# HeyWeCome/WhisprRec

Hardware: AMD Instinct MI355X
Metric: BPR training triplets/sec (higher is better)
Workload: dtype f32; 1 GPU; BPRMF emb_size=64, synthetic 1000000 users x 1000000 items (uniform ids), batch 65536, SGD l2=0, plan build in timed region; batch=65536, emb_size=64, optimizer=SGD, plan_chunk_batches=64, tables=single GPU, step_stream=whisprrec_amd.hip_ops.PipelinedSgd, plan=group plan (no per-batch sort: flags + lists of the shared rows, wr_group.hip), chained_step_launch=True, plan_build=on a side stream, beside the steps of the chunk before

## Files before the change

whisprrec_amd/csrc/wr_group.hip:

```cpp
#include "wr_common.h"
#include <hip/hip_ext.h>

#include <algorithm>

namespace wr {

constexpr int kGpThreads = 1024;
constexpr unsigned kGpRangeBits = 18;
constexpr int kGpWords = 1 << (kGpRangeBits - 5);
constexpr int kGpCap = 8192;
constexpr int kGpBins = 4096;
constexpr int kGpMaxBin = 256;
constexpr int kGpMaxRanges = 8;
constexpr int64_t kGpMaxBatch = 1 << 17;
constexpr int kGpLongRun = 64;
constexpr int kGpMetaWords = 16;
#ifndef WR_GP_DBG
#define WR_GP_DBG 0
#endif

struct GroupLayout {
    int64_t nb, B, fw;
    int R_u, R_i, cap_u, cap_i;
    unsigned mask_u, mask_i, hbits_u, hbits_i;
    int64_t flags, ucnt, icnt, ul_row, ul_src, il_row, il_src, total;
    int64_t zero_words;
};

static inline int ranges_for(int64_t n_rows, unsigned *mask, unsigned *hbits, int *cap) {
    unsigned bits = kGpRangeBits;
    while (bits < kGpRangeBits + 3 && (int64_t(1) << bits) < n_rows) ++bits;
    *mask = (1u << bits) - 1u;
    *hbits = bits;
    const int R = 1 << (bits - kGpRangeBits);
    *cap = kGpCap;
    return R;
}

static bool group_layout(int64_t n, int64_t B, int64_t n_users, int64_t n_items, GroupLayout &L) {
    if (n <= 0 || n >= (int64_t(1) << 31) || B <= 0 || B > kGpMaxBatch) return false;
    if (n_users <= 0 || n_users >= (int64_t(1) << 31) || n_items <= 0 || n_items >= (int64_t(1) << 31)) return false;
    L.nb = (n + B - 1) / B;
    L.B = B;
    L.fw = (B + 31) / 32;
    L.R_u = ranges_for(n_users, &L.mask_u, &L.hbits_u, &L.cap_u);
    L.R_i = ranges_for(n_items, &L.mask_i, &L.hbits_i, &L.cap_i);
    L.flags = kGpMetaWords;
    L.ucnt = L.flags + L.nb * L.fw * 4;
    L.icnt = L.ucnt + align_up(L.nb * L.R_u, 4);
    L.zero_words = L.icnt + align_up(L.nb * L.R_i, 4);
    L.ul_row = L.zero_words;
    L.ul_src = L.ul_row + L.nb * L.R_u * (int64_t)L.cap_u;
    L.il_row = L.ul_src + L.nb * L.R_u * (int64_t)L.cap_u;
    L.il_src = L.il_row + L.nb * L.R_i * (int64_t)L.cap_i;
    L.total = L.il_src + L.nb * L.R_i * (int64_t)L.cap_i;
    return true;
}

struct GpDev {
    int *meta;
    unsigned *flags;
    int *ucnt, *icnt;
    int *ul_row, *ul_src, *il_row, *il_src;
    int R_u, R_i, cap_u, cap_i;
    unsigned mask_u, mask_i, hbits_u, hbits_i;
    int fw;
};

static inline GpDev group_dev(int32_t *plan, const GroupLayout &L) {
    return GpDev{plan, reinterpret_cast<unsigned *>(plan + L.flags), plan + L.ucnt, plan + L.icnt, plan + L.ul_row,
                 plan + L.ul_src, plan + L.il_row, plan + L.il_src, L.R_u, L.R_i, L.cap_u, L.cap_i, L.mask_u, L.mask_i,
                 L.hbits_u, L.hbits_i, (int)L.fw};
}

template <typename F>
__device__ __forceinline__ void gp_scan(const int *__restrict__ a, int cnt, F f) {
    if ((reinterpret_cast<uintptr_t>(a) & 15u) == 0) {
        const int n4 = cnt >> 2;
        const int4 *a4 = reinterpret_cast<const int4 *>(a);
        int i = threadIdx.x;
        for (; i + 3 * kGpThreads < n4; i += 4 * kGpThreads) {
            int4 v[4];
#pragma unroll
            for (int q = 0; q < 4; ++q) v[q] = a4[i + q * kGpThreads];
#pragma unroll
            for (int q = 0; q < 4; ++q) {
                const int at = 4 * (i + q * kGpThreads);
                f(v[q].x, at);
                f(v[q].y, at + 1);
                f(v[q].z, at + 2);
                f(v[q].w, at + 3);
            }
        }
        for (; i < n4; i += kGpThreads) {
            const int4 v = a4[i];
            f(v.x, 4 * i);
            f(v.y, 4 * i + 1);
            f(v.z, 4 * i + 2);
            f(v.w, 4 * i + 3);
        }
        for (int j = (n4 << 2) + threadIdx.x; j < cnt; j += kGpThreads) f(a[j], j);
    } else {
        for (int j = threadIdx.x; j < cnt; j += kGpThreads) f(a[j], j);
    }
}

__global__ __launch_bounds__(kGpThreads) void group_plan_kernel(const int *__restrict__ u, const int *__restrict__ p,
                                                                 const int *__restrict__ n, int64_t n_total, int B, int nb,
                                                                 int n_users, int n_items, GpDev L) {
    extern __shared__ __attribute__((aligned(16))) unsigned gp_lds[];
    unsigned *seen = gp_lds;
    unsigned long long *keys = reinterpret_cast<unsigned long long *>(gp_lds);
    unsigned *multi = gp_lds + 2 * kGpCap;
    unsigned *f0 = multi + kGpWords, *f1 = f0 + L.fw, *f2 = f1 + L.fw;
    int &n_list = *reinterpret_cast<int *>(f2 + L.fw);
    const int per = L.R_u + L.R_i;
    const unsigned lb = xcd_contiguous_id(blockIdx.x, gridDim.x);
    const int b = (int)(lb / (unsigned)per), rr = (int)(lb % (unsigned)per);
    const bool item = rr >= L.R_u;
    const unsigned r = (unsigned)(item ? rr - L.R_u : rr);
    const int64_t base = (int64_t)b * B;
    const int Bb = (int)((base + B <= n_total) ? B : (n_total - base));
    const unsigned n_rows = (unsigned)(item ? n_items : n_users);
    const unsigned mask = item ? L.mask_i : L.mask_u;
    const unsigned rb = (item ? L.hbits_i : L.hbits_u) - kGpRangeBits, rsel = (1u << rb) - 1u;
    for (int i = threadIdx.x; i < kGpWords; i += kGpThreads) {
        seen[i] = 0u;
        multi[i] = 0u;
    }
    for (int i = threadIdx.x; i < 3 * L.fw; i += kGpThreads) f0[i] = 0u;
    if (threadIdx.x == 0) n_list = 0;
    __syncthreads();
    auto mark = [&](int row, int) {
        if ((unsigned)row >= n_rows) {
            L.meta[0] = 1;
            return;
        }
        const unsigned h = (unsigned)row & mask;
        if ((h & rsel) != r) return;
        const unsigned bit = h >> rb, m = 1u << (bit & 31u);
        const unsigned old = atomicOr(&seen[bit >> 5], m);
        if (old & m) atomicOr(&multi[bit >> 5], m);
    };
    if (!(WR_GP_DBG & 8)) {
        if (item) {
            gp_scan(p + base, Bb, mark);
            gp_scan(n + base, Bb, mark);
        } else {
            gp_scan(u + base, Bb, mark);
        }
    }
    __syncthreads();
    auto several = [&](int row) -> bool {
        const unsigned h = (unsigned)row & mask;
        if ((h & rsel) != r) return false;
        const unsigned bit = h >> rb;
        return (multi[bit >> 5] >> (bit & 31u)) & 1u;
    };
    auto append = [&](int row, unsigned src) {
        const int pos = atomicAdd(&n_list, 1);
        if (pos < kGpCap) keys[pos] = ((unsigned long long)(unsigned)row << 32) | src;
    };
    if (!(WR_GP_DBG & 2)) {
        const bool next = b + 1 < nb && !(WR_GP_DBG & 16);
        const int64_t nbase = base + B;
        const int Bn = next ? (int)((nbase + B <= n_total) ? B : (n_total - nbase)) : 0;
        auto defer = [&](int row, int t) {
            if (several(row)) atomicOr(&f2[t >> 5], 1u << (t & 31));
        };
        if (item) {
            gp_scan(p + base, Bb, [&](int row, int t) {
                if (several(row)) {
                    atomicOr(&f0[t >> 5], 1u << (t & 31));
                    append(row, (unsigned)t << 1);
                }
            });
            gp_scan(n + base, Bb, [&](int row, int t) {
                if (several(row)) {
                    atomicOr(&f1[t >> 5], 1u << (t & 31));
                    append(row, ((unsigned)t << 1) | 1u);
                }
            });
            gp_scan(p + nbase, Bn, defer);
            gp_scan(n + nbase, Bn, defer);
        } else {
            gp_scan(u + base, Bb, [&](int row, int t) {
                if (several(row)) {
                    atomicOr(&f0[t >> 5], 1u << (t & 31));
                    append(row, (unsigned)t << 1);
                }
            });
            gp_scan(u + nbase, Bn, defer);
        }
    }
    __syncthreads();
    if (!(WR_GP_DBG & 4)) {
        unsigned *fb = L.flags + (int64_t)b * L.fw * 4;
        for (int w = threadIdx.x; w < L.fw; w += kGpThreads) {
            if (f0[w]) __hip_atomic_fetch_or(fb + 4 * w + (item ? 1 : 0), f0[w], __ATOMIC_RELAXED, __HIP_MEMORY_SCOPE_AGENT);
            if (item && f1[w]) __hip_atomic_fetch_or(fb + 4 * w + 2, f1[w], __ATOMIC_RELAXED, __HIP_MEMORY_SCOPE_AGENT);
            if (f2[w])
                __hip_atomic_fetch_or(fb + 4 * (L.fw + w) + 3, f2[w], __ATOMIC_RELAXED, __HIP_MEMORY_SCOPE_AGENT);
        }
    }
    const int cap = item ? L.cap_i : L.cap_u, R = item ? L.R_i : L.R_u;
    int m = n_list;
    if (m > cap) {
        if (threadIdx.x == 0) L.meta[1] = 1;
        m = cap;
    }
    int *cnt = reinterpret_cast<int *>(multi);
    unsigned short *out16 = reinterpret_cast<unsigned short *>(multi + kGpBins);
    int *wave_tot = reinterpret_cast<int *>(f0);
    auto bin_of = [&](unsigned long long k) -> int { return (int)(((((unsigned)(k >> 32)) & mask) >> rb) & (kGpBins - 1)); };
    int *lrow = (item ? L.il_row : L.ul_row) + ((int64_t)b * R + r) * cap, *lsrc = (item ? L.il_src : L.ul_src) + ((int64_t)b * R + r) * cap;
    __syncthreads();
    for (int i = threadIdx.x; i < kGpBins; i += kGpThreads) cnt[i] = 0;
    __syncthreads();
    if (!(WR_GP_DBG & 1)) {
        for (int j = threadIdx.x; j < m; j += kGpThreads) atomicAdd(&cnt[bin_of(keys[j])], 1);
        __syncthreads();
        constexpr int kOwn = kGpBins / kGpThreads;
        const int c0 = (int)threadIdx.x * kOwn;
        int local = 0;
#pragma unroll
        for (int j = 0; j < kOwn; ++j) local += cnt[c0 + j];
        int incl = local;
#pragma unroll
        for (int d = 1; d < 64; d <<= 1) {
            const int v = __shfl_up(incl, d, 64);
            if ((int)(threadIdx.x & 63) >= d) incl += v;
        }
        if ((threadIdx.x & 63) == 63) wave_tot[threadIdx.x >> 6] = incl;
        __syncthreads();
        int run = incl - local;
        for (int w = 0; w < (int)(threadIdx.x >> 6); ++w) run += wave_tot[w];
#pragma unroll
        for (int j = 0; j < kOwn; ++j) {
            const int c = cnt[c0 + j];
            cnt[c0 + j] = run;
            run += c;
        }
        __syncthreads();
        for (int j = threadIdx.x; j < m; j += kGpThreads) out16[atomicAdd(&cnt[bin_of(keys[j])], 1)] = (unsigned short)j;
        __syncthreads();
        for (int j = threadIdx.x; j < m; j += kGpThreads) {
            const unsigned long long k = keys[j];
            const int bin = bin_of(k);
            const int lo = bin ? cnt[bin - 1] : 0, hi = cnt[bin];
            if (hi - lo > kGpMaxBin) {
                L.meta[1] = 1;
                continue;
            }
            int pos = lo, same = 0;
            for (int jj = lo; jj < hi; ++jj) {
                const unsigned long long o = keys[out16[jj]];
                pos += o < k ? 1 : 0;
                same += (unsigned)(o >> 32) == (unsigned)(k >> 32) ? 1 : 0;
            }
            if (same > kGpLongRun) L.meta[2] = 1;
            lrow[pos] = (int)(k >> 32);
            lsrc[pos] = (int)(unsigned)k;
        }
    } else {
        for (int j = threadIdx.x; j < m; j += kGpThreads) {
            lrow[j] = (int)(keys[j] >> 32);
            lsrc[j] = (int)(unsigned)keys[j];
        }
    }
    if (threadIdx.x == 0) (item ? L.icnt : L.ucnt)[(int64_t)b * R + r] = m;
}

__global__ __launch_bounds__(kBlock) void narrow_ids_kernel(const int64_t *__restrict__ u, const int64_t *__restrict__ p,
                                                             const int64_t *__restrict__ n, int *__restrict__ u32,
                                                             int *__restrict__ p32, int *__restrict__ n32, int64_t cnt) {
    const int64_t i = (int64_t)blockIdx.x * kBlock + threadIdx.x;
    if (i >= cnt) return;
    const int64_t a = u[i], b = p[i], c = n[i];
    u32[i] = (a >= 0 && a < (int64_t(1) << 31)) ? (int)a : -1;
    p32[i] = (b >= 0 && b < (int64_t(1) << 31)) ? (int)b : -1;
    n32[i] = (c >= 0 && c < (int64_t(1) << 31)) ? (int)c : -1;
}

constexpr int kGsTile = 32;
constexpr int kGsAhead = 8;
constexpr int kGsShards = 64;
constexpr int kGsShardStride = 16;
constexpr int kGsStepWords = kGsShards * kGsShardStride;
constexpr int kGsDefChunk = 32;
constexpr int kGsLdsInts = 1024 + 8;
constexpr unsigned kGsSpinLimit = 1u << 22;

struct GsBatch {
    const int *u, *p, *n;
    const uint4 *flags;
    const int *ul_row, *ul_src, *ul_cnt, *il_row, *il_src, *il_cnt;
    int B, R_u, R_i, cap_u, cap_i;
};

struct GsArgs {
    float *U, *I;
    int D;
    float lr;
    GsBatch cur;
    float *Z, *ZU, *partials;
    float denom;
    GsBatch prev;
    const float *Zp, *ZUp, *partials_prev;
    int n_partials_prev;
    float denom_prev;
    float *loss_prev;
    int nA, nIT, nUT, nDS, tiles_at, side_at;
    int chained;
    unsigned *done, *timeout;
    float *Gs;
    int nL;
};

template <int NV>
__device__ __forceinline__ Row<NV> row_zero() {
    Row<NV> r;
#pragma unroll
    for (int k = 0; k < NV; ++k) r.v[k] = make_float4(0.f, 0.f, 0.f, 0.f);
    return r;
}

template <int T, int NV, bool FULL>
__device__ __forceinline__ void gs_single(const GsArgs &a, int t, int u, int p, int n, bool us, bool ps, bool ns, int lane,
                                          float &terms) {
    const Row<NV> ur = load_row<T, NV, FULL>(a.U, u, a.D, lane);
    const Row<NV> pr = load_row<T, NV, FULL>(a.I, p, a.D, lane);
    const Row<NV> nr = load_row<T, NV, FULL>(a.I, n, a.D, lane);
    const float sp = team_sum<T>(dot_partial<NV>(ur, pr));
    const float sn = team_sum<T>(dot_partial<NV>(ur, nr));
    float term, c;
    bpr_terms(sp, sn, a.denom, term, c);
    terms += term;
    Row<NV> g, z;
#pragma unroll
    for (int k = 0; k < NV; ++k) {
        g.v[k] = make_float4(c * (pr.v[k].x - nr.v[k].x), c * (pr.v[k].y - nr.v[k].y), c * (pr.v[k].z - nr.v[k].z),
                             c * (pr.v[k].w - nr.v[k].w));
        z.v[k] = make_float4(c * ur.v[k].x, c * ur.v[k].y, c * ur.v[k].z, c * ur.v[k].w);
    }
    const float lr = a.lr;
    if (!us) {
        Row<NV> w;
#pragma unroll
        for (int k = 0; k < NV; ++k)
            w.v[k] = make_float4(ur.v[k].x - lr * g.v[k].x, ur.v[k].y - lr * g.v[k].y, ur.v[k].z - lr * g.v[k].z,
                                 ur.v[k].w - lr * g.v[k].w);
        store_row<T, NV, FULL>(a.U, u, a.D, lane, w);
    } else {
        store_row<T, NV, FULL>(a.ZU, t, a.D, lane, g);
    }
    if (!ps) {
        if (a.Gs != nullptr && p >= a.nL) {
            store_row<T, NV, FULL>(a.Gs, p - a.nL, a.D, lane, z);
        } else {
            Row<NV> w;
#pragma unroll
            for (int k = 0; k < NV; ++k)
                w.v[k] = make_float4(pr.v[k].x - lr * z.v[k].x, pr.v[k].y - lr * z.v[k].y, pr.v[k].z - lr * z.v[k].z,
                                     pr.v[k].w - lr * z.v[k].w);
            store_row<T, NV, FULL>(a.I, p, a.D, lane, w);
        }
    }
    if (!ns) {
        if (a.Gs != nullptr && n >= a.nL) {
            Row<NV> zn;
#pragma unroll
            for (int k = 0; k < NV; ++k) zn.v[k] = make_float4(-z.v[k].x, -z.v[k].y, -z.v[k].z, -z.v[k].w);
            store_row<T, NV, FULL>(a.Gs, n - a.nL, a.D, lane, zn);
        } else {
            Row<NV> w;
#pragma unroll
            for (int k = 0; k < NV; ++k)
                w.v[k] = make_float4(nr.v[k].x - lr * (-z.v[k].x), nr.v[k].y - lr * (-z.v[k].y), nr.v[k].z - lr * (-z.v[k].z),
                                     nr.v[k].w - lr * (-z.v[k].w));
            store_row<T, NV, FULL>(a.I, n, a.D, lane, w);
        }
    }
    if (ps || ns) store_row<T, NV, FULL>(a.Z, t, a.D, lane, z);
}

__device__ __forceinline__ void gs_wait_tiles(const GsArgs &a) {
    if (threadIdx.x < 64) {
        const int j = (int)threadIdx.x;
        const int n_sig = a.nIT + a.nUT;
        const unsigned want = j < kGsShards ? (unsigned)((n_sig - j + kGsShards - 1) / kGsShards) : 0u;
        const unsigned *shard = a.done + (j < kGsShards ? j : 0) * kGsShardStride;
        unsigned spins = 0;
        for (;;) {
            const bool ok = __hip_atomic_load(shard, __ATOMIC_RELAXED, __HIP_MEMORY_SCOPE_AGENT) >= want;
            if (__all(ok)) break;
            __builtin_amdgcn_s_sleep(8);
            if (++spins > kGsSpinLimit) {
                if (j == 0) __hip_atomic_store(a.timeout, 1u, __ATOMIC_RELAXED, __HIP_MEMORY_SCOPE_AGENT);
                break;
            }
        }
        __builtin_amdgcn_fence(__ATOMIC_ACQUIRE, "agent");
        asm volatile("s_waitcnt vmcnt(0)" ::: "memory");
    }
    __syncthreads();
}

__device__ __forceinline__ bool gs_tile_of(const int *__restrict__ cnt, int R, int cap, int q, int &seg, int &e0, int &len) {
    int c[kGpMaxRanges];
#pragma unroll
    for (int s = 0; s < kGpMaxRanges; ++s) c[s] = cnt[s < R ? s : 0];
    asm volatile("" : "+v"(c[0]), "+v"(c[1]), "+v"(c[2]), "+v"(c[3]), "+v"(c[4]), "+v"(c[5]), "+v"(c[6]), "+v"(c[7]));
#pragma unroll
    for (int s = 0; s < kGpMaxRanges; ++s)
        if (s >= R) c[s] = 0;
    bool found = false;
#pragma unroll
    for (int s = 0; s < kGpMaxRanges; ++s) {
        const int cs = min(c[s], cap);
        const int nt = (cs + kGsTile - 1) / kGsTile;
        if (!found && q < nt) {
// ... 240 lines not shown
#if WR_GS_DBG & 8
        f = make_uint4(0u, 0u, 0u, 0u);
#endif
        asm volatile("" : "+v"(u), "+v"(p), "+v"(n), "+v"(f.x), "+v"(f.y), "+v"(f.z), "+v"(f.w));
        const unsigned bit = 1u << (t & 31);
        if (t < a.cur.B && !(a.chained && (f.w & bit)))
            gs_single<T, NV, FULL>(a, t, u, p, n, f.x & bit, f.y & bit, f.z & bit, lane, terms);
        slot = b;
    }
    if (lane != 0) terms = 0.f;
    const float sum = block_sum(terms, scratch);
    if (threadIdx.x == 0) a.partials[slot] = sum;
}

static inline int64_t gs_ws_one(int64_t B, int32_t D) {
    const int64_t nA = (B + teams_per_block(D) - 1) / teams_per_block(D);
    return 2 * align_up(B * (int64_t)D * 4, 256) + align_up((nA + 512) * 4, 256);
}

#ifndef WR_GS_TILES_AT
#define WR_GS_TILES_AT 0
#endif
#ifndef WR_GS_SIDE_AT
#define WR_GS_SIDE_AT 12
#endif
#ifndef WR_GS_NUT
#define WR_GS_NUT 256
#endif
#ifndef WR_GS_NDS
#define WR_GS_NDS 64
#endif
#ifndef WR_GS_NIT
#define WR_GS_NIT 1024
#endif

struct GroupRun {
    TablePair tabs;
    const int32_t *u, *p, *n, *plan;
    int64_t n_triplets, batch_size, plan_words, workspace_bytes, sync_words;
    BatchRange range;
    float lr, *loss_out;
    void *const *events;
    void *workspace;
    uint32_t *sync;
    int n_cu;
    float *grad_slots;
    int64_t n_local_items, global_batch;
    hipStream_t stream;
};

template <int T, int NV, bool FULL>
static int32_t launch_group_steps(const GroupRun &g, const GroupLayout &L, const GpDev &G) {
    const int32_t D = g.tabs.D;
    const int64_t n_batches = g.range.n_batches, global_batch = g.global_batch;
    uint32_t *const sync = g.sync;
    const int64_t B = L.B;
    const int64_t ws_one = gs_ws_one(B, D), zb = align_up(B * (int64_t)D * 4, 256);
    char *ws = reinterpret_cast<char *>(g.workspace);
    float *Zs[2] = {reinterpret_cast<float *>(ws), reinterpret_cast<float *>(ws + ws_one)};
    float *ZUs[2] = {reinterpret_cast<float *>(ws + zb), reinterpret_cast<float *>(ws + ws_one + zb)};
    float *Ps[2] = {reinterpret_cast<float *>(ws + 2 * zb), reinterpret_cast<float *>(ws + ws_one + 2 * zb)};
    constexpr int TEAMS = kBlock / T;
    WR_HIP(hipMemsetAsync(sync, 0, (size_t)(n_batches * kGsStepWords) * 4, g.stream));
    uint32_t *timeout = sync + (g.sync_words - 4);
    int nDS = WR_GS_NDS;
    while (nDS > g.n_cu / 4 && nDS > 1) nDS >>= 1;
    auto batch_of = [&](int64_t b) {
        const int64_t off = b * B;
        const int Bk = (int)batch_len(g.n_triplets, B, b);
        return GsBatch{g.u + off, g.p + off, g.n + off, reinterpret_cast<const uint4 *>(G.flags + b * L.fw * 4),
                       G.ul_row + b * L.R_u * (int64_t)L.cap_u, G.ul_src + b * L.R_u * (int64_t)L.cap_u, G.ucnt + b * L.R_u,
                       G.il_row + b * L.R_i * (int64_t)L.cap_i, G.il_src + b * L.R_i * (int64_t)L.cap_i, G.icnt + b * L.R_i,
                       Bk, L.R_u, L.R_i, L.cap_u, L.cap_i};
    };
    auto ev = [&](int64_t k, int j) { return g.events ? reinterpret_cast<hipEvent_t>(g.events[2 * k + j]) : (hipEvent_t) nullptr; };
    int n_partials_prev = 0;
    for (int64_t k = 0; k <= n_batches; ++k) {
        GsArgs a{};
        a.U = g.tabs.U;
        a.I = g.tabs.I;
        a.D = D;
        a.lr = g.lr;
        a.done = sync + (k < n_batches ? k : 0) * kGsStepWords;
        a.timeout = timeout;
        a.Gs = g.grad_slots;
        a.nL = (int)g.n_local_items;
        const bool have_cur = k < n_batches, have_prev = k > 0;
        if (have_cur) {
            a.cur = batch_of(g.range.first_batch + k);
            a.Z = Zs[k & 1];
            a.ZU = ZUs[k & 1];
            a.partials = Ps[k & 1];
            a.denom = global_batch > 0 ? (float)global_batch : (float)a.cur.B;
            a.nA = (int)((a.cur.B + TEAMS - 1) / TEAMS);
            a.nDS = have_prev ? nDS : 0;
            a.chained = have_prev ? 1 : 0;
        }
        if (have_prev) {
            a.prev = batch_of(g.range.first_batch + k - 1);
            a.Zp = Zs[(k - 1) & 1];
            a.ZUp = ZUs[(k - 1) & 1];
            a.partials_prev = Ps[(k - 1) & 1];
            a.n_partials_prev = n_partials_prev;
            a.denom_prev = global_batch > 0 ? (float)global_batch : (float)a.prev.B;
            a.loss_prev = at_or_null(g.loss_out, k - 1);
            a.nIT = (int)std::min<int64_t>(WR_GS_NIT, (2 * B + kGsTile - 1) / kGsTile + L.R_i);
            a.nUT = (int)std::min<int64_t>(WR_GS_NUT, (B + kGsTile - 1) / kGsTile + L.R_u);
        }
        a.tiles_at = (int)((int64_t)a.nA * WR_GS_TILES_AT / 16);
        a.side_at = std::max(a.tiles_at, (int)((int64_t)a.nA * WR_GS_SIDE_AT / 16));
        const dim3 grid((unsigned)(a.nA + a.nIT + a.nUT + a.nDS));
        hipEvent_t e0 = have_cur ? ev(k, 0) : nullptr, e1 = have_cur ? ev(k, 1) : nullptr;
        if (e0 != nullptr || e1 != nullptr)
            hipExtLaunchKernelGGL((bprmf_group_step<T, NV, FULL>), grid, dim3(kBlock), 0, g.stream, e0, e1, 0, a);
        else
            hipLaunchKernelGGL((bprmf_group_step<T, NV, FULL>), grid, dim3(kBlock), 0, g.stream, a);
        WR_LAUNCH_CHECK("bprmf_group_step");
        n_partials_prev = a.nA + a.nDS;
    }
    return WR_OK;
}

static int32_t check_group_plan(const char *entry, const GroupRun &g, GroupLayout &L) {
    int32_t rc;
    if ((rc = check_whole_lines(entry, whole_lines(g.tabs.U, g.tabs.I, g.tabs.D), g.tabs.D)) != WR_OK) return rc;
    WR_REQUIRE(group_layout(g.n_triplets, g.batch_size, g.tabs.n_users, g.tabs.n_items, L), WR_E_RANGE,
               "group plan not applicable to n=%lld, batch=%lld", (long long)g.n_triplets, (long long)g.batch_size);
    WR_REQUIRE(g.plan_words >= L.total, WR_E_WORKSPACE, "group plan: %lld words < %lld", (long long)g.plan_words, (long long)L.total);
    return WR_OK;
}

static int32_t run_group(const char *entry, GroupRun &g, const GroupLayout &L, int64_t sync_batches) {
    int32_t rc;
    if ((rc = check_workspace(entry, g.workspace, g.workspace_bytes, 2 * gs_ws_one(g.batch_size, g.tabs.D))) != WR_OK) return rc;
    if ((rc = check_sync_words(entry, g.sync, g.sync_words, sync_batches * kGsStepWords + 4)) != WR_OK) return rc;
    if (g.range.n_batches == 0) return WR_OK;
    if (g.n_cu == 0 && (rc = device_cu_count(&g.n_cu)) != WR_OK) return rc;
    const GpDev G = group_dev(const_cast<int32_t *>(g.plan), L);
#define WR_CALL_GS(T_, NV_, FULL_) return launch_group_steps<T_, NV_, FULL_>(g, L, G)
    WR_DISPATCH_D(g.tabs.D, WR_CALL_GS);
#undef WR_CALL_GS
    return WR_OK;
}

}

using namespace wr;

extern "C" {

int64_t wr_group_plan_words(int64_t n_triplets, int64_t batch_size, int64_t n_users, int64_t n_items) {
    GroupLayout L;
    if (!group_layout(n_triplets, batch_size, n_users, n_items, L)) return 0;
    return L.total;
}

int32_t wr_group_plan_layout(int64_t n_triplets, int64_t batch_size, int64_t n_users, int64_t n_items, int64_t *out) {
    WR_REQUIRE(out != nullptr, WR_E_NULL, "out is NULL");
    GroupLayout L;
    WR_REQUIRE(group_layout(n_triplets, batch_size, n_users, n_items, L), WR_E_RANGE,
               "group plan not applicable to n=%lld, batch=%lld", (long long)n_triplets, (long long)batch_size);
    const int64_t v[16] = {L.nb, L.fw, L.R_u, L.R_i, (int64_t)L.mask_u, (int64_t)L.mask_i, L.flags, L.ucnt, L.icnt, L.ul_row,
                           L.ul_src, L.il_row, L.il_src, L.total, L.cap_u, L.cap_i};
    for (int i = 0; i < 16; ++i) out[i] = v[i];
    return WR_OK;
}

int32_t wr_narrow_ids_i64(const int64_t *u, const int64_t *p, const int64_t *n, int32_t *u32, int32_t *p32, int32_t *n32,
                          int64_t count, void *stream_) {
    WR_REQUIRE(u && p && n && u32 && p32 && n32, WR_E_NULL, "index arrays must not be NULL");
    WR_REQUIRE(count >= 0 && count < (int64_t(1) << 40), WR_E_SHAPE, "count out of range");
    if (count == 0) return WR_OK;
    hipLaunchKernelGGL(narrow_ids_kernel, dim3((unsigned)((count + kBlock - 1) / kBlock)), dim3(kBlock), 0,
                       reinterpret_cast<hipStream_t>(stream_), u, p, n, u32, p32, n32, count);
    WR_LAUNCH_CHECK("narrow_ids_kernel");
    return WR_OK;
}

int32_t wr_group_plan_build(const int32_t *u, const int32_t *p, const int32_t *n, int64_t n_triplets, int64_t batch_size,
                            int64_t n_users, int64_t n_items, int32_t *plan, int64_t plan_words, void *stream_) {
    WR_REQUIRE(u && p && n && plan, WR_E_NULL, "index arrays / plan must not be NULL");
    GroupLayout L;
    WR_REQUIRE(group_layout(n_triplets, batch_size, n_users, n_items, L), WR_E_RANGE,
               "group plan not applicable to n=%lld, batch=%lld", (long long)n_triplets, (long long)batch_size);
    WR_REQUIRE(aligned16(plan) && plan_words >= L.total, WR_E_WORKSPACE, "group plan: %lld words < %lld", (long long)plan_words,
               (long long)L.total);
    WR_REQUIRE(L.nb * (L.R_u + L.R_i) < (int64_t(1) << 31), WR_E_SHAPE, "group plan: too many batches in one plan");
    hipStream_t stream = reinterpret_cast<hipStream_t>(stream_);
    WR_HIP(hipMemsetAsync(plan, 0, (size_t)L.zero_words * 4, stream));
    const size_t lds = (size_t)(2 * kGpCap + kGpWords + 3 * L.fw + 4) * 4;
    static bool attr_set = false;
    if (!attr_set) {
        WR_HIP(hipFuncSetAttribute(reinterpret_cast<const void *>(group_plan_kernel), hipFuncAttributeMaxDynamicSharedMemorySize,
                                   (int)((2 * kGpCap + kGpWords + 3 * ((kGpMaxBatch + 31) / 32) + 4) * 4)));
        attr_set = true;
    }
    const GpDev G = group_dev(plan, L);
    hipLaunchKernelGGL(group_plan_kernel, dim3((unsigned)(L.nb * (L.R_u + L.R_i))), dim3(kGpThreads), lds, stream, u, p, n,
                       n_triplets, (int)batch_size, (int)L.nb, (int)n_users, (int)n_items, G);
    WR_LAUNCH_CHECK("group_plan_kernel");
    return WR_OK;
}

int64_t wr_bprmf_group_workspace_bytes(int64_t batch_size, int32_t D) { return 2 * gs_ws_one(batch_size, D); }

int64_t wr_bprmf_group_sync_words(int64_t n_batches) { return n_batches < 0 ? WR_E_SHAPE : (n_batches + 1) * kGsStepWords + 4; }

int32_t wr_bprmf_group_supported(const float *user_tab, const float *item_tab, int32_t D) {
    return (user_tab && item_tab && D >= 4 && D <= 1024 && D % 4 == 0 && whole_lines(user_tab, item_tab, D)) ? 1 : 0;
}

int32_t wr_bprmf_run_sgd_group(float *user_tab, int64_t n_users, float *item_tab, int64_t n_items, int32_t D,
                               const int32_t *u, const int32_t *p, const int32_t *n, int64_t n_triplets, int64_t batch_size,
                               const int32_t *plan, int64_t plan_words, int64_t first_batch, int64_t n_batches, float lr,
                               float *loss_out, void *const *events, void *workspace, int64_t workspace_bytes, int32_t *sync,
                               int64_t sync_words, void *stream) {
    GroupRun g{};
    g.tabs = TablePair{user_tab, item_tab, n_users, n_items, D};
    g.u = u; g.p = p; g.n = n; g.n_triplets = n_triplets; g.batch_size = batch_size;
    g.plan = plan; g.plan_words = plan_words;
    g.range = BatchRange{first_batch, n_batches};
    g.lr = lr; g.loss_out = loss_out; g.events = events;
    g.workspace = workspace; g.workspace_bytes = workspace_bytes;
    g.sync = reinterpret_cast<uint32_t *>(sync); g.sync_words = sync_words;
    g.stream = reinterpret_cast<hipStream_t>(stream);
    int32_t rc;
    GroupLayout L;
    if ((rc = check_tables(g.tabs)) != WR_OK) return rc;
    WR_REQUIRE(u && p && n && plan && sync, WR_E_NULL, "index arrays / plan / sync words must not be NULL");
    if ((rc = check_group_plan("wr_bprmf_run_sgd_group", g, L)) != WR_OK) return rc;
    WR_REQUIRE(first_batch >= 0 && n_batches >= 0 && first_batch + n_batches <= L.nb, WR_E_SHAPE,
               "batches [%lld,%lld) exceed the plan's %lld", (long long)first_batch, (long long)(first_batch + n_batches),
               (long long)L.nb);
    return run_group("wr_bprmf_run_sgd_group", g, L, n_batches + 1);
}

int32_t wr_bprmf_shard_step_group(float *user_shard, int64_t n_user_rows, float *item_ext, int64_t n_ext_rows,
                                  int64_t n_local_items, int32_t D, const int32_t *vu, const int32_t *vp, const int32_t *vn,
                                  int64_t n_triplets, int64_t batch_size, const int32_t *plan, int64_t plan_words, int64_t batch,
                                  int64_t global_batch, float lr, float *grad_slots, float *loss_partial, void *workspace,
                                  int64_t workspace_bytes, int32_t *sync, int64_t sync_words, void *stream) {
    GroupRun g{};
    g.tabs = TablePair{user_shard, item_ext, n_user_rows, n_ext_rows, D};
    g.u = vu; g.p = vp; g.n = vn; g.n_triplets = n_triplets; g.batch_size = batch_size;
    g.plan = plan; g.plan_words = plan_words;
    g.range = BatchRange{batch, 1};
    g.lr = lr; g.loss_out = loss_partial;
    g.workspace = workspace; g.workspace_bytes = workspace_bytes;
    g.sync = reinterpret_cast<uint32_t *>(sync); g.sync_words = sync_words;
    g.n_cu = 256;
    g.grad_slots = grad_slots; g.n_local_items = n_local_items; g.global_batch = global_batch;
    g.stream = reinterpret_cast<hipStream_t>(stream);
    int32_t rc;
    GroupLayout L;
    if ((rc = check_tables(g.tabs, "user_shard", "item_ext")) != WR_OK) return rc;
    WR_REQUIRE(vu && vp && vn && plan && sync && grad_slots, WR_E_NULL, "index arrays / plan / sync words / grad_slots must not be NULL");
    WR_REQUIRE(aligned16(grad_slots), WR_E_ALIGN, "grad_slots is not 16-byte aligned");
    WR_REQUIRE(n_local_items >= 0 && n_local_items <= n_ext_rows, WR_E_SHAPE, "n_local_items %lld outside [0, %lld]",
               (long long)n_local_items, (long long)n_ext_rows);
    if ((rc = check_group_plan("wr_bprmf_shard_step_group", g, L)) != WR_OK) return rc;
    WR_REQUIRE(batch >= 0 && batch < L.nb, WR_E_SHAPE, "batch %lld outside the plan's %lld", (long long)batch, (long long)L.nb);
    WR_REQUIRE(global_batch >= batch_size, WR_E_SHAPE, "global_batch %lld < local batch %lld", (long long)global_batch,
               (long long)batch_size);
    return run_group("wr_bprmf_shard_step_group", g, L, 2);
}

}
```

Baseline: 2.590 billion triplets/s.

## Add per-range bucket deal pass ahead of group plan range kernel

Adds a group_deal_kernel that scatters each batch's user and item ids into per-range buckets, so every range block would scan only its own rows instead of the whole batch. That kernel also zeroes the flag and count words and does the id range check, which replaces the large plan memset. The range kernel now works on range-local bit indices and rebuilds full row ids afterwards, with a deeper unrolled vector scan. As written, bucket_cap returns 0 for every R >= 1, so the bucket path never runs; the rest is an extra launch plus a reworked scan and zeroing, with a dormant code path to maintain.

```diff
diff --git a/whisprrec_amd/csrc/wr_group.hip b/whisprrec_amd/csrc/wr_group.hip
--- a/whisprrec_amd/csrc/wr_group.hip
+++ b/whisprrec_amd/csrc/wr_group.hip
@@ -15,16 +15,17 @@
 constexpr int64_t kGpMaxBatch = 1 << 17;
 constexpr int kGpLongRun = 64;
 constexpr int kGpMetaWords = 16;
-#ifndef WR_GP_DBG
-#define WR_GP_DBG 0
-#endif
+constexpr int kGdThreads = 256;
+constexpr int kGdPer = 8;
+constexpr int kGdSpan = kGdThreads * kGdPer;
 
 struct GroupLayout {
     int64_t nb, B, fw;
     int R_u, R_i, cap_u, cap_i;
     unsigned mask_u, mask_i, hbits_u, hbits_i;
     int64_t flags, ucnt, icnt, ul_row, ul_src, il_row, il_src, total;
-    int64_t zero_words;
+    int bcap_u, bcap_i;
+    int64_t bcnt, ub, ib, words;
 };
 
 static inline int ranges_for(int64_t n_rows, unsigned *mask, unsigned *hbits, int *cap) {
@@ -35,6 +36,11 @@
     const int R = 1 << (bits - kGpRangeBits);
     *cap = kGpCap;
     return R;
+}
+
+static inline int bucket_cap(int64_t occ, int R) {
+    if (R >= 1) return 0;
+    return (int)align_up(std::min<int64_t>(occ, occ / R * 5 / 4 + 1024), 4);
 }
 
 static bool group_layout(int64_t n, int64_t B, int64_t n_users, int64_t n_items, GroupLayout &L) {
@@ -48,12 +54,17 @@
     L.flags = kGpMetaWords;
     L.ucnt = L.flags + L.nb * L.fw * 4;
     L.icnt = L.ucnt + align_up(L.nb * L.R_u, 4);
-    L.zero_words = L.icnt + align_up(L.nb * L.R_i, 4);
-    L.ul_row = L.zero_words;
+    L.ul_row = L.icnt + align_up(L.nb * L.R_i, 4);
     L.ul_src = L.ul_row + L.nb * L.R_u * (int64_t)L.cap_u;
     L.il_row = L.ul_src + L.nb * L.R_u * (int64_t)L.cap_u;
     L.il_src = L.il_row + L.nb * L.R_i * (int64_t)L.cap_i;
     L.total = L.il_src + L.nb * L.R_i * (int64_t)L.cap_i;
+    L.bcap_u = bucket_cap(B, L.R_u);
+    L.bcap_i = bucket_cap(2 * B, L.R_i);
+    L.bcnt = L.total;
+    L.ub = L.bcnt + ((L.bcap_u | L.bcap_i) ? align_up(L.nb * (L.R_u + L.R_i), 4) : 0);
+    L.ib = L.ub + L.nb * L.R_u * 2 * (int64_t)L.bcap_u;
+    L.words = L.ib + L.nb * L.R_i * 2 * (int64_t)L.bcap_i;
     return true;
 }
 
@@ -65,49 +76,219 @@
     int R_u, R_i, cap_u, cap_i;
     unsigned mask_u, mask_i, hbits_u, hbits_i;
     int fw;
+    int *bcnt, *ub, *ib;
+    int bcap_u, bcap_i;
 };
 
 static inline GpDev group_dev(int32_t *plan, const GroupLayout &L) {
     return GpDev{plan, reinterpret_cast<unsigned *>(plan + L.flags), plan + L.ucnt, plan + L.icnt, plan + L.ul_row,
                  plan + L.ul_src, plan + L.il_row, plan + L.il_src, L.R_u, L.R_i, L.cap_u, L.cap_i, L.mask_u, L.mask_i,
-                 L.hbits_u, L.hbits_i, (int)L.fw};
-}
-
-template <typename F>
-__device__ __forceinline__ void gp_scan(const int *__restrict__ a, int cnt, F f) {
-    if ((reinterpret_cast<uintptr_t>(a) & 15u) == 0) {
-        const int n4 = cnt >> 2;
-        const int4 *a4 = reinterpret_cast<const int4 *>(a);
-        int i = threadIdx.x;
-        for (; i + 3 * kGpThreads < n4; i += 4 * kGpThreads) {
-            int4 v[4];
-#pragma unroll
-            for (int q = 0; q < 4; ++q) v[q] = a4[i + q * kGpThreads];
-#pragma unroll
-            for (int q = 0; q < 4; ++q) {
+                 L.hbits_u, L.hbits_i, (int)L.fw, plan + L.bcnt, plan + L.ub, plan + L.ib, L.bcap_u, L.bcap_i};
+}
+
+__device__ __forceinline__ void gd_count(unsigned long long &lo, unsigned long long &hi, unsigned r) {
+    if (r < 4u) lo += 1ull << (16u * r);
+    else hi += 1ull << (16u * (r - 4u));
+}
+
+__device__ __forceinline__ unsigned gd_field(unsigned long long lo, unsigned long long hi, unsigned r) {
+    return (unsigned)((r < 4u ? lo >> (16u * r) : hi >> (16u * (r - 4u))) & 0xffffull);
+}
+
+__global__ __launch_bounds__(kGdThreads) void group_deal_kernel(const int *__restrict__ u, const int *__restrict__ p,
+                                                                 const int *__restrict__ n, int64_t n_total, int B, int nb,
+                                                                 int spans, int n_users, int n_items, GpDev L) {
+    __shared__ unsigned long long wave_tot[kGdThreads / 64][4];
+    __shared__ int gbase[2 * kGpMaxRanges], rstart[2 * kGpMaxRanges];
+    __shared__ int stage[4 * kGdSpan];
+    const int b = (int)(blockIdx.x / (unsigned)spans), t0 = (int)(blockIdx.x % (unsigned)spans) * kGdSpan;
+    const int64_t base = (int64_t)b * B;
+    const int Bb = (int)((base + B <= n_total) ? B : (n_total - base));
+    const int tid = (int)threadIdx.x, lane = tid & 63, wave = tid >> 6;
+    {
+        uint4 *fb = reinterpret_cast<uint4 *>(L.flags) + (int64_t)b * L.fw;
+        const int w = t0 / 32 + tid;
+        if (tid < kGdSpan / 32 && w < L.fw) fb[w] = make_uint4(0u, 0u, 0u, 0u);
+        if (blockIdx.x == 0 && tid < 4) {
+            const int64_t eu = (int64_t)nb * L.R_u + tid, ei = (int64_t)nb * L.R_i + tid;
+            if (eu < (((int64_t)nb * L.R_u + 3) & ~int64_t(3))) L.ucnt[eu] = 0;
+            if (ei < (((int64_t)nb * L.R_i + 3) & ~int64_t(3))) L.icnt[ei] = 0;
+        }
+    }
+    const int *ub = u + base, *pb = p + base, *nbk = n + base;
+    const bool vec = ((reinterpret_cast<uintptr_t>(ub) | reinterpret_cast<uintptr_t>(pb) | reinterpret_cast<uintptr_t>(nbk)) & 15u) == 0;
+    int iu[kGdPer], ip[kGdPer], in[kGdPer];
+#pragma unroll
+    for (int q = 0; q < kGdPer / 4; ++q) {
+        const int t = t0 + 4 * (tid + q * kGdThreads);
+        if (vec && t + 3 < Bb) {
+            const int4 a = *reinterpret_cast<const int4 *>(ub + t), c = *reinterpret_cast<const int4 *>(pb + t),
+                       d = *reinterpret_cast<const int4 *>(nbk + t);
+            iu[4 * q] = a.x, iu[4 * q + 1] = a.y, iu[4 * q + 2] = a.z, iu[4 * q + 3] = a.w;
+            ip[4 * q] = c.x, ip[4 * q + 1] = c.y, ip[4 * q + 2] = c.z, ip[4 * q + 3] = c.w;
+            in[4 * q] = d.x, in[4 * q + 1] = d.y, in[4 * q + 2] = d.z, in[4 * q + 3] = d.w;
+        } else {
+#pragma unroll
+            for (int j = 0; j < 4; ++j) {
+                const bool ok = t + j < Bb;
+                iu[4 * q + j] = ok ? ub[t + j] : 0;
+                ip[4 * q + j] = ok ? pb[t + j] : 0;
+                in[4 * q + j] = ok ? nbk[t + j] : 0;
+            }
+        }
+    }
+    const unsigned rsel_u = (unsigned)L.R_u - 1u, rsel_i = (unsigned)L.R_i - 1u;
+    const unsigned rb_u = L.hbits_u - kGpRangeBits, rb_i = L.hbits_i - kGpRangeBits;
+    const bool deal_u = L.bcap_u != 0, deal_i = L.bcap_i != 0;
+    unsigned long long c[4] = {0ull, 0ull, 0ull, 0ull};
+    bool bad = false;
+#pragma unroll
+    for (int k = 0; k < kGdPer; ++k) {
+        const int t = t0 + 4 * (tid + (k >> 2) * kGdThreads) + (k & 3);
+        if (t < Bb) {
+            const unsigned a = (unsigned)iu[k], pp = (unsigned)ip[k], nn = (unsigned)in[k];
+            if (a >= (unsigned)n_users) bad = true;
+            else if (deal_u) gd_count(c[0], c[1], a & rsel_u);
+            if (pp >= (unsigned)n_items) bad = true;
+            else if (deal_i) gd_count(c[2], c[3], pp & rsel_i);
+            if (nn >= (unsigned)n_items) bad = true;
+            else if (deal_i) gd_count(c[2], c[3], nn & rsel_i);
+        }
+    }
+    if (bad) L.meta[0] = 1;
+    if (!deal_u && !deal_i) return;
+    unsigned long long ex[4], tot[4];
+#pragma unroll
+    for (int k = 0; k < 4; ++k) {
+        unsigned long long incl = c[k];
+#pragma unroll
+        for (int d = 1; d < 64; d <<= 1) {
+            const unsigned long long v = __shfl_up(incl, d, 64);
+            if (lane >= d) incl += v;
+        }
+        if (lane == 63) wave_tot[wave][k] = incl;
+        ex[k] = incl - c[k];
+    }
+    __syncthreads();
+#pragma unroll
+    for (int k = 0; k < 4; ++k) {
+        tot[k] = 0ull;
+#pragma unroll
+        for (int w = 0; w < kGdThreads / 64; ++w) {
+            if (w == wave) ex[k] += tot[k];
+            tot[k] += wave_tot[w][k];
+        }
+    }
+    const int per = L.R_u + L.R_i;
+    if (tid < per) {
+        const bool item = tid >= L.R_u;
+        const unsigned r = (unsigned)(item ? tid - L.R_u : tid);
+        const unsigned long long lo = item ? tot[2] : tot[0], hi = item ? tot[3] : tot[1];
+        const int cnt = (int)gd_field(lo, hi, r);
+        int first = 0;
+        for (unsigned q = 0; q < r; ++q) first += (int)gd_field(lo, hi, q);
+        int at = 0;
+        if (cnt > 0) {
+            at = atomicAdd(&L.bcnt[(int64_t)b * per + tid], cnt);
+            if (at + cnt > (item ? L.bcap_i : L.bcap_u)) L.meta[1] = 1;
+        }
+        const int g = item ? kGpMaxRanges + (int)r : (int)r;
+        gbase[g] = at;
+        rstart[g] = first;
+    }
+    __syncthreads();
+    auto place = [&](unsigned h, unsigned rsel, unsigned rb, int g0, unsigned long long &lo, unsigned long long &hi, unsigned src) {
+        const unsigned r = h & rsel;
+        const int at = rstart[g0 + (int)r] + (int)gd_field(lo, hi, r);
+        gd_count(lo, hi, r);
+        stage[at] = (int)(h >> rb);
+        stage[2 * kGdSpan + at] = (int)src;
+    };
+    auto copy_out = [&](int *bk, int bcap, int R, int g0, int total) {
+        __syncthreads();
+        for (int i = tid; i < total; i += kGdThreads) {
+            int r = 0;
+            for (int q = 1; q < R; ++q) r += i >= rstart[g0 + q] ? 1 : 0;
+            const int slot = gbase[g0 + r] + i - rstart[g0 + r];
+            if (slot < bcap) {
+                int *q = bk + (int64_t)r * 2 * bcap;
+                q[slot] = stage[i];
+                q[bcap + slot] = stage[2 * kGdSpan + i];
+            }
+        }
+        __syncthreads();
+    };
+    if (deal_u) {
+#pragma unroll
+        for (int k = 0; k < kGdPer; ++k) {
+            const int t = t0 + 4 * (tid + (k >> 2) * kGdThreads) + (k & 3);
+            const unsigned a = (unsigned)iu[k];
+            if (t < Bb && a < (unsigned)n_users) place(a & L.mask_u, rsel_u, rb_u, 0, ex[0], ex[1], (unsigned)t << 1);
+        }
+        int total = 0;
+        for (int r = 0; r < L.R_u; ++r) total += (int)gd_field(tot[0], tot[1], (unsigned)r);
+        copy_out(L.ub + (int64_t)b * L.R_u * 2 * L.bcap_u, L.bcap_u, L.R_u, 0, total);
+    }
+    if (deal_i) {
+#pragma unroll
+        for (int k = 0; k < kGdPer; ++k) {
+            const int t = t0 + 4 * (tid + (k >> 2) * kGdThreads) + (k & 3);
+            const unsigned pp = (unsigned)ip[k], nn = (unsigned)in[k];
+            if (t < Bb && pp < (unsigned)n_items) place(pp & L.mask_i, rsel_i, rb_i, kGpMaxRanges, ex[2], ex[3], (unsigned)t << 1);
+            if (t < Bb && nn < (unsigned)n_items) place(nn & L.mask_i, rsel_i, rb_i, kGpMaxRanges, ex[2], ex[3], ((unsigned)t << 1) | 1u);
+        }
+        int total = 0;
+        for (int r = 0; r < L.R_i; ++r) total += (int)gd_field(tot[2], tot[3], (unsigned)r);
+        copy_out(L.ib + (int64_t)b * L.R_i * 2 * L.bcap_i, L.bcap_i, L.R_i, kGpMaxRanges, total);
+    }
+}
+
+struct GpSeg {
+    const int *a, *s;
+    int cnt;
+    unsigned mask, neg;
+};
+
+template <int U, bool SRC, typename F>
+__device__ __forceinline__ void gp_scan(const GpSeg &g, F f) {
+    const bool pairs = g.s != nullptr;
+    auto one = [&](int v, int sv, int j) {
+        if (pairs) f((unsigned)v & (unsigned)(kGpWords * 32 - 1), (unsigned)sv);
+        else f((unsigned)v & g.mask, ((unsigned)j << 1) | g.neg);
+    };
+    if (g.cnt <= 0) return;
+    if (((reinterpret_cast<uintptr_t>(g.a) | reinterpret_cast<uintptr_t>(g.s)) & 15u) == 0) {
+        const int n4 = g.cnt >> 2;
+        const int4 *a4 = reinterpret_cast<const int4 *>(g.a), *s4 = reinterpret_cast<const int4 *>(g.s);
+        for (int i = threadIdx.x; i < n4; i += U * kGpThreads) {
+            int4 v[U], sv[U];
+#pragma unroll
+            for (int q = 0; q < U; ++q) {
+                const int at = min(i + q * kGpThreads, n4 - 1);
+                v[q] = a4[at];
+                sv[q] = make_int4(0, 0, 0, 0);
+                if (SRC && pairs) sv[q] = s4[at];
+            }
+#pragma unroll
+            for (int q = 0; q < U; ++q) {
                 const int at = 4 * (i + q * kGpThreads);
-                f(v[q].x, at);
-                f(v[q].y, at + 1);
-                f(v[q].z, at + 2);
-                f(v[q].w, at + 3);
-            }
-        }
-        for (; i < n4; i += kGpThreads) {
-            const int4 v = a4[i];
-            f(v.x, 4 * i);
-            f(v.y, 4 * i + 1);
-            f(v.z, 4 * i + 2);
-            f(v.w, 4 * i + 3);
-        }
-        for (int j = (n4 << 2) + threadIdx.x; j < cnt; j += kGpThreads) f(a[j], j);
+                if (i + q * kGpThreads < n4) {
+                    one(v[q].x, sv[q].x, at);
+                    one(v[q].y, sv[q].y, at + 1);
+                    one(v[q].z, sv[q].z, at + 2);
+                    one(v[q].w, sv[q].w, at + 3);
+                }
+            }
+        }
+        for (int j = (n4 << 2) + threadIdx.x; j < g.cnt; j += kGpThreads) one(g.a[j], (SRC && pairs) ? g.s[j] : 0, j);
     } else {
-        for (int j = threadIdx.x; j < cnt; j += kGpThreads) f(a[j], j);
-    }
-}
-
-__global__ __launch_bounds__(kGpThreads) void group_plan_kernel(const int *__restrict__ u, const int *__restrict__ p,
-                                                                 const int *__restrict__ n, int64_t n_total, int B, int nb,
-                                                                 int n_users, int n_items, GpDev L) {
+        for (int j = threadIdx.x; j < g.cnt; j += kGpThreads) one(g.a[j], (SRC && pairs) ? g.s[j] : 0, j);
+    }
+}
+
+__global__ __launch_bounds__(kGpThreads) void group_range_kernel(const int *__restrict__ u, const int *__restrict__ p,
+                                                                  const int *__restrict__ n, int64_t n_total, int B, int nb,
+                                                                  int n_users, int n_items, GpDev L) {
     extern __shared__ __attribute__((aligned(16))) unsigned gp_lds[];
     unsigned *seen = gp_lds;
     unsigned long long *keys = reinterpret_cast<unsigned long long *>(gp_lds);
@@ -120,10 +301,28 @@
     const bool item = rr >= L.R_u;
     const unsigned r = (unsigned)(item ? rr - L.R_u : rr);
     const int64_t base = (int64_t)b * B;
-    const int Bb = (int)((base + B <= n_total) ? B : (n_total - base));
     const unsigned n_rows = (unsigned)(item ? n_items : n_users);
     const unsigned mask = item ? L.mask_i : L.mask_u;
-    const unsigned rb = (item ? L.hbits_i : L.hbits_u) - kGpRangeBits, rsel = (1u << rb) - 1u;
+    const unsigned rb = (item ? L.hbits_i : L.hbits_u) - kGpRangeBits;
+    const int R = item ? L.R_i : L.R_u, bcap = item ? L.bcap_i : L.bcap_u;
+    auto segs_of = [&](int k, GpSeg &s0, GpSeg &s1) {
+        const int64_t kb = (int64_t)k * B;
+        const int Bk = (int)((kb + B <= n_total) ? B : (n_total - kb));
+        s1 = GpSeg{nullptr, nullptr, 0, mask, 1u};
+        if (bcap != 0) {
+            const int *bk = (item ? L.ib : L.ub) + ((int64_t)k * R + r) * 2 * bcap;
+            s0 = GpSeg{bk, bk + bcap, min(L.bcnt[(int64_t)k * per + rr], bcap), mask, 0u};
+        } else if (item) {
+            s0 = GpSeg{p + kb, nullptr, Bk, mask, 0u};
+            s1 = GpSeg{n + kb, nullptr, Bk, mask, 1u};
+        } else {
+            s0 = GpSeg{u + kb, nullptr, Bk, mask, 0u};
+        }
+    };
+    GpSeg own0, own1, nxt0, nxt1;
+    segs_of(b, own0, own1);
+    nxt0 = nxt1 = GpSeg{nullptr, nullptr, 0, mask, 0u};
+    if (b + 1 < nb) segs_of(b + 1, nxt0, nxt1);
     for (int i = threadIdx.x; i < kGpWords; i += kGpThreads) {
         seen[i] = 0u;
         multi[i] = 0u;
@@ -131,70 +330,33 @@
     for (int i = threadIdx.x; i < 3 * L.fw; i += kGpThreads) f0[i] = 0u;
     if (threadIdx.x == 0) n_list = 0;
     __syncthreads();
-    auto mark = [&](int row, int) {
-        if ((unsigned)row >= n_rows) {
-            L.meta[0] = 1;
-            return;
-        }
-        const unsigned h = (unsigned)row & mask;
-        if ((h & rsel) != r) return;
-        const unsigned bit = h >> rb, m = 1u << (bit & 31u);
+    auto mark = [&](unsigned bit, unsigned) {
+        const unsigned m = 1u << (bit & 31u);
         const unsigned old = atomicOr(&seen[bit >> 5], m);
         if (old & m) atomicOr(&multi[bit >> 5], m);
     };
-    if (!(WR_GP_DBG & 8)) {
-        if (item) {
-            gp_scan(p + base, Bb, mark);
-            gp_scan(n + base, Bb, mark);
-        } else {
-            gp_scan(u + base, Bb, mark);
-        }
-    }
-    __syncthreads();
-    auto several = [&](int row) -> bool {
-        const unsigned h = (unsigned)row & mask;
-        if ((h & rsel) != r) return false;
-        const unsigned bit = h >> rb;
-        return (multi[bit >> 5] >> (bit & 31u)) & 1u;
+    gp_scan<8, false>(own0, mark);
+    gp_scan<8, false>(own1, mark);
+    __syncthreads();
+    auto several = [&](unsigned bit) -> bool { return (multi[bit >> 5] >> (bit & 31u)) & 1u; };
+    auto shared = [&](unsigned bit, unsigned src) {
+        if (several(bit)) {
+            const unsigned t = min(src >> 1, (unsigned)B - 1u);
+            atomicOr(&((src & 1u) ? f1 : f0)[t >> 5], 1u << (t & 31u));
+            const int pos = atomicAdd(&n_list, 1);
+            if (pos < kGpCap) keys[pos] = ((unsigned long long)bit << 32) | src;
+        }
     };
-    auto append = [&](int row, unsigned src) {
-        const int pos = atomicAdd(&n_list, 1);
-        if (pos < kGpCap) keys[pos] = ((unsigned long long)(unsigned)row << 32) | src;
+    auto defer = [&](unsigned bit, unsigned src) {
+        const unsigned t = min(src >> 1, (unsigned)B - 1u);
+        if (several(bit)) atomicOr(&f2[t >> 5], 1u << (t & 31u));
     };
-    if (!(WR_GP_DBG & 2)) {
-        const bool next = b + 1 < nb && !(WR_GP_DBG & 16);
-        const int64_t nbase = base + B;
-        const int Bn = next ? (int)((nbase + B <= n_total) ? B : (n_total - nbase)) : 0;
-        auto defer = [&](int row, int t) {
-            if (several(row)) atomicOr(&f2[t >> 5], 1u << (t & 31));
-        };
-        if (item) {
-            gp_scan(p + base, Bb, [&](int row, int t) {
-                if (several(row)) {
-                    atomicOr(&f0[t >> 5], 1u << (t & 31));
-                    append(row, (unsigned)t << 1);
-                }
-            });
-            gp_scan(n + base, Bb, [&](int row, int t) {
-                if (several(row)) {
-                    atomicOr(&f1[t >> 5], 1u << (t & 31));
-                    append(row, ((unsigned)t << 1) | 1u);
-                }
-            });
-            gp_scan(p + nbase, Bn, defer);
-            gp_scan(n + nbase, Bn, defer);
-        } else {
-            gp_scan(u + base, Bb, [&](int row, int t) {
-                if (several(row)) {
-                    atomicOr(&f0[t >> 5], 1u << (t & 31));
-                    append(row, (unsigned)t << 1);
-                }
-            });
-            gp_scan(u + nbase, Bn, defer);
-        }
-    }
-    __syncthreads();
-    if (!(WR_GP_DBG & 4)) {
+    gp_scan<8, true>(own0, shared);
+    gp_scan<8, true>(own1, shared);
+    gp_scan<8, true>(nxt0, defer);
+    gp_scan<8, true>(nxt1, defer);
+    __syncthreads();
+    {
         unsigned *fb = L.flags + (int64_t)b * L.fw * 4;
         for (int w = threadIdx.x; w < L.fw; w += kGpThreads) {
             if (f0[w]) __hip_atomic_fetch_or(fb + 4 * w + (item ? 1 : 0), f0[w], __ATOMIC_RELAXED, __HIP_MEMORY_SCOPE_AGENT);
@@ -203,11 +365,35 @@
                 __hip_atomic_fetch_or(fb + 4 * (L.fw + w) + 3, f2[w], __ATOMIC_RELAXED, __HIP_MEMORY_SCOPE_AGENT);
         }
     }
-    const int cap = item ? L.cap_i : L.cap_u, R = item ? L.R_i : L.R_u;
+    const int cap = item ? L.cap_i : L.cap_u;
     int m = n_list;
     if (m > cap) {
         if (threadIdx.x == 0) L.meta[1] = 1;
         m = cap;
+    }
+    if (n_rows > mask + 1u) {
+        constexpr int kOwnKeys = kGpCap / kGpThreads;
+        int row[kOwnKeys];
+#pragma unroll
+        for (int q = 0; q < kOwnKeys; ++q) {
+            const int j = (int)threadIdx.x + q * kGpThreads;
+            row[q] = 0;
+            if (j < m) {
+                const unsigned src = (unsigned)keys[j];
+                const unsigned t = min(src >> 1, (unsigned)B - 1u);
+                row[q] = (item ? ((src & 1u) ? n : p) : u)[base + t];
+            }
+        }
+#pragma unroll
+        for (int q = 0; q < kOwnKeys; ++q) {
+            const int j = (int)threadIdx.x + q * kGpThreads;
+            if (j < m) keys[j] = ((unsigned long long)(unsigned)row[q] << 32) | (unsigned)keys[j];
+        }
+    } else {
+        for (int j = threadIdx.x; j < m; j += kGpThreads) {
+            const unsigned long long k = keys[j];
+            keys[j] = ((unsigned long long)((((unsigned)(k >> 32)) << rb) | r) << 32) | (unsigned)k;
+        }
     }
     int *cnt = reinterpret_cast<int *>(multi);
     unsigned short *out16 = reinterpret_cast<unsigned short *>(multi + kGpBins);
@@ -217,56 +403,49 @@
     __syncthreads();
     for (int i = threadIdx.x; i < kGpBins; i += kGpThreads) cnt[i] = 0;
     __syncthreads();
-    if (!(WR_GP_DBG & 1)) {
-        for (int j = threadIdx.x; j < m; j += kGpThreads) atomicAdd(&cnt[bin_of(keys[j])], 1);
-        __syncthreads();
-        constexpr int kOwn = kGpBins / kGpThreads;
-        const int c0 = (int)threadIdx.x * kOwn;
-        int local = 0;
-#pragma unroll
-        for (int j = 0; j < kOwn; ++j) local += cnt[c0 + j];
-        int incl = local;
-#pragma unroll
-        for (int d = 1; d < 64; d <<= 1) {
-            const int v = __shfl_up(incl, d, 64);
-            if ((int)(threadIdx.x & 63) >= d) incl += v;
-        }
-        if ((threadIdx.x & 63) == 63) wave_tot[threadIdx.x >> 6] = incl;
-        __syncthreads();
-        int run = incl - local;
-        for (int w = 0; w < (int)(threadIdx.x >> 6); ++w) run += wave_tot[w];
-#pragma unroll
-        for (int j = 0; j < kOwn; ++j) {
-            const int c = cnt[c0 + j];
-            cnt[c0 + j] = run;
-            run += c;
-        }
-        __syncthreads();
-        for (int j = threadIdx.x; j < m; j += kGpThreads) out16[atomicAdd(&cnt[bin_of(keys[j])], 1)] = (unsigned short)j;
-        __syncthreads();
-        for (int j = threadIdx.x; j < m; j += kGpThreads) {
-            const unsigned long long k = keys[j];
-            const int bin = bin_of(k);
-            const int lo = bin ? cnt[bin - 1] : 0, hi = cnt[bin];
-            if (hi - lo > kGpMaxBin) {
-                L.meta[1] = 1;
-                continue;
-            }
-            int pos = lo, same = 0;
-            for (int jj = lo; jj < hi; ++jj) {
-                const unsigned long long o = keys[out16[jj]];
-                pos += o < k ? 1 : 0;
-                same += (unsigned)(o >> 32) == (unsigned)(k >> 32) ? 1 : 0;
-            }
-            if (same > kGpLongRun) L.meta[2] = 1;
-            lrow[pos] = (int)(k >> 32);
-            lsrc[pos] = (int)(unsigned)k;
-        }
-    } else {
-        for (int j = threadIdx.x; j < m; j += kGpThreads) {
-            lrow[j] = (int)(keys[j] >> 32);
-            lsrc[j] = (int)(unsigned)keys[j];
-        }
+    for (int j = threadIdx.x; j < m; j += kGpThreads) atomicAdd(&cnt[bin_of(keys[j])], 1);
+    __syncthreads();
+    constexpr int kOwn = kGpBins / kGpThreads;
+    const int c0 = (int)threadIdx.x * kOwn;
+    int local = 0;
+#pragma unroll
+    for (int j = 0; j < kOwn; ++j) local += cnt[c0 + j];
+    int incl = local;
+#pragma unroll
+    for (int d = 1; d < 64; d <<= 1) {
+        const int v = __shfl_up(incl, d, 64);
+        if ((int)(threadIdx.x & 63) >= d) incl += v;
+    }
+    if ((threadIdx.x & 63) == 63) wave_tot[threadIdx.x >> 6] = incl;
+    __syncthreads();
+    int run = incl - local;
+    for (int w = 0; w < (int)(threadIdx.x >> 6); ++w) run += wave_tot[w];
+#pragma unroll
+    for (int j = 0; j < kOwn; ++j) {
+        const int c = cnt[c0 + j];
+        cnt[c0 + j] = run;
+        run += c;
+    }
+    __syncthreads();
+    for (int j = threadIdx.x; j < m; j += kGpThreads) out16[atomicAdd(&cnt[bin_of(keys[j])], 1)] = (unsigned short)j;
+    __syncthreads();
+    for (int j = threadIdx.x; j < m; j += kGpThreads) {
+        const unsigned long long k = keys[j];
+        const int bin = bin_of(k);
+        const int lo = bin ? cnt[bin - 1] : 0, hi = cnt[bin];
+        if (hi - lo > kGpMaxBin) {
+            L.meta[1] = 1;
+            continue;
+        }
+        int pos = lo, same = 0;
+        for (int jj = lo; jj < hi; ++jj) {
+            const unsigned long long o = keys[out16[jj]];
+            pos += o < k ? 1 : 0;
+            same += (unsigned)(o >> 32) == (unsigned)(k >> 32) ? 1 : 0;
+        }
+        if (same > kGpLongRun) L.meta[2] = 1;
+        lrow[pos] = (int)(k >> 32);
+        lsrc[pos] = (int)(unsigned)k;
     }
     if (threadIdx.x == 0) (item ? L.icnt : L.ucnt)[(int64_t)b * R + r] = m;
 }
@@ -813,7 +992,7 @@
 int64_t wr_group_plan_words(int64_t n_triplets, int64_t batch_size, int64_t n_users, int64_t n_items) {
     GroupLayout L;
     if (!group_layout(n_triplets, batch_size, n_users, n_items, L)) return 0;
-    return L.total;
+    return L.words;
 }
 
 int32_t wr_group_plan_layout(int64_t n_triplets, int64_t batch_size, int64_t n_users, int64_t n_items, int64_t *out) {
@@ -844,22 +1023,32 @@
     GroupLayout L;
     WR_REQUIRE(group_layout(n_triplets, batch_size, n_users, n_items, L), WR_E_RANGE,
                "group plan not applicable to n=%lld, batch=%lld", (long long)n_triplets, (long long)batch_size);
-    WR_REQUIRE(aligned16(plan) && plan_words >= L.total, WR_E_WORKSPACE, "group plan: %lld words < %lld", (long long)plan_words,
-               (long long)L.total);
+    WR_REQUIRE(aligned16(plan) && plan_words >= L.words, WR_E_WORKSPACE, "group plan: %lld words < %lld", (long long)plan_words,
+               (long long)L.words);
     WR_REQUIRE(L.nb * (L.R_u + L.R_i) < (int64_t(1) << 31), WR_E_SHAPE, "group plan: too many batches in one plan");
     hipStream_t stream = reinterpret_cast<hipStream_t>(stream_);
-    WR_HIP(hipMemsetAsync(plan, 0, (size_t)L.zero_words * 4, stream));
+    WR_HIP(hipMemsetAsync(plan, 0, (size_t)kGpMetaWords * 4, stream));
+    if (L.ub > L.bcnt) WR_HIP(hipMemsetAsync(plan + L.bcnt, 0, (size_t)(L.ub - L.bcnt) * 4, stream));
     const size_t lds = (size_t)(2 * kGpCap + kGpWords + 3 * L.fw + 4) * 4;
-    static bool attr_set = false;
-    if (!attr_set) {
-        WR_HIP(hipFuncSetAttribute(reinterpret_cast<const void *>(group_plan_kernel), hipFuncAttributeMaxDynamicSharedMemorySize,
-                                   (int)((2 * kGpCap + kGpWords + 3 * ((kGpMaxBatch + 31) / 32) + 4) * 4)));
-        attr_set = true;
+    {
+        constexpr int kMaxDev = 64;
+        static bool attr_set[kMaxDev] = {};
+        int dev = 0;
+        WR_HIP(hipGetDevice(&dev));
+        if (dev < 0 || dev >= kMaxDev || !attr_set[dev]) {
+            WR_HIP(hipFuncSetAttribute(reinterpret_cast<const void *>(group_range_kernel), hipFuncAttributeMaxDynamicSharedMemorySize,
+                                       (int)((2 * kGpCap + kGpWords + 3 * ((kGpMaxBatch + 31) / 32) + 4) * 4)));
+            if (dev >= 0 && dev < kMaxDev) attr_set[dev] = true;
+        }
     }
     const GpDev G = group_dev(plan, L);
-    hipLaunchKernelGGL(group_plan_kernel, dim3((unsigned)(L.nb * (L.R_u + L.R_i))), dim3(kGpThreads), lds, stream, u, p, n,
+    const int64_t spans = (batch_size + kGdSpan - 1) / kGdSpan;
+    hipLaunchKernelGGL(group_deal_kernel, dim3((unsigned)(L.nb * spans)), dim3(kGdThreads), 0, stream, u, p, n, n_triplets,
+                       (int)batch_size, (int)L.nb, (int)spans, (int)n_users, (int)n_items, G);
+    WR_LAUNCH_CHECK("group_deal_kernel");
+    hipLaunchKernelGGL(group_range_kernel, dim3((unsigned)(L.nb * (L.R_u + L.R_i))), dim3(kGpThreads), lds, stream, u, p, n,
                        n_triplets, (int)batch_size, (int)L.nb, (int)n_users, (int)n_items, G);
-    WR_LAUNCH_CHECK("group_plan_kernel");
+    WR_LAUNCH_CHECK("group_range_kernel");
     return WR_OK;
 }
 
```

Result: slower. 2.264 billion triplets/s (-12.6%).
